# sina-behnam/RTSDS

Hardware: AMD Instinct MI355X
Metric: images/sec/node (train step) + inference FPS@1024x512, BiSeNet 19-cls (higher is better)
Workload: dtype bf16; 1 GPU; configs[1]: BiSeNet-R18 seg-only train step (train.py:65-113); model=BiSeNet-ResNet18, global_batch=8, per_gpu_batch=8, image=3x512x1024, num_classes=19, parallelism=dp1

## Files before the change

### include/rtsds_hip.h

```cpp
#ifndef RTSDS_HIP_H
#define RTSDS_HIP_H
#include <stddef.h>
#include <stdint.h>
#ifdef __cplusplus
extern "C" {
#endif

enum { RTSDS_F32 = 0, RTSDS_BF16 = 1, RTSDS_F16 = 2  };
enum {
  RTSDS_OK = 0,
  RTSDS_ERR_SHAPE = 1,
  RTSDS_ERR_UNSUPPORTED = 2,
  RTSDS_ERR_LAUNCH = 3,
  RTSDS_ERR_WORKSPACE = 4
};
enum { RTSDS_ACT_NONE = 0, RTSDS_ACT_RELU = 1, RTSDS_ACT_LEAKY = 2, RTSDS_ACT_SIGMOID = 3 };
#define RTSDS_ACCUMULATE 0x100
#define RTSDS_INPUT_PADDED 0x400
#define RTSDS_WEIGHT_PACKED 0x800

typedef struct {
  int n, h, w, c;
  int ho, wo, k;
  int kh, kw;
// ... 255 lines not shown

int rtsds_graph_split(void* graph, int max_lanes, void** handle, int* n_segments, int* n_lanes);
int rtsds_graph_lanes(void* graph, int max_lanes);
int rtsds_graph_nodes(void* graph);
int rtsds_capture_nodes(void* stream);
int rtsds_graph_split_launch(void* handle, void* stream);
int rtsds_graph_split_destroy(void* handle);

int rtsds_pooled_mlp_bwd(const void* da, const void* a, const void* h, const void* p, const void* w1,
                         const void* w2, float* dw1, float* db1, float* dw2, float* db2, void* dp,
                         int n, int c0, int c1, int c2, int accumulate, int dtype, void* stream);

int rtsds_pooled_mlp_fwd(const void* p, const void* w1, const float* b1, const void* w2, const float* b2, void* h,
                         void* a, int n, int c0, int c1, int c2, int dtype, void* stream);

#define RTSDS_ABI_VERSION 21
int rtsds_abi_version(void);

#ifdef __cplusplus
}
#endif
#endif
```

### rtsds_amd/_lib.py

```python
import ctypes
import os

import torch

_HERE = os.path.dirname(os.path.abspath(__file__))
DEFAULT_LIB_PATH = os.path.join(_HERE, "librtsds_hip.so")
ABI_VERSION = 21
LIB_PATH = os.environ.get("RTSDS_LIB") or DEFAULT_LIB_PATH

F32, BF16 = 0, 1
ACT_NONE, ACT_RELU, ACT_LEAKY, ACT_SIGMOID = 0, 1, 2, 3
ACCUMULATE = 0x100
INPUT_PADDED = 0x400
WEIGHT_PACKED = 0x800
UPCE_SET_CORRECT = 2
ERRORS = {1: "bad shape", 2: "unsupported configuration", 3: "HIP launch failure", 4: "workspace too small"}

c_int, c_long, c_float, c_size_t, c_void_p = (ctypes.c_int, ctypes.c_long, ctypes.c_float,
                                              ctypes.c_size_t, ctypes.c_void_p)


class ConvDesc(ctypes.Structure):
    _fields_ = [(n, c_int) for n in ("n", "h", "w", "c", "ho", "wo", "k", "kh", "kw", "sh", "sw",
                                     "ph", "pw", "dh", "dw", "dtype")]
# ... 27 lines not shown
                                            ctypes.POINTER(SplitReduceDesc), P]),
    "rtsds_split_reduce_many": (c_int, [c_int, ctypes.POINTER(SplitReduceDesc), P]),
    "rtsds_imgconv_bn_wgrad_workspace": (c_size_t, [ctypes.POINTER(ConvDesc)]),
    "rtsds_imgconv_bn_wgrad": (c_int, [ctypes.POINTER(ConvDesc), P, P, P, P, c_int, P, c_int, P, c_size_t, P]),
    "rtsds_imgconv_bn_wgrad_deferred": (c_int, [ctypes.POINTER(ConvDesc), P, P, P, P, c_int, P, c_int, P, c_size_t,
                                                ctypes.POINTER(SplitReduceDesc), P]),
    "rtsds_bn_workspace": (c_size_t, [c_long, c_int]),
    "rtsds_bn_bwd_coef": (c_int, [P, P, P, P, P, c_long, c_int, P, P, P, P, c_int, c_int, c_int, c_int, P, c_size_t, P]),
    "rtsds_bn_fwd": (c_int, [P, P, P, c_long, c_int, P, P, P, P, P, P, P, c_float, c_float, c_int,
                             c_int, P, c_int, c_int, P, c_size_t, P]),
    "rtsds_bn_fwd_ld": (c_int, [P, P, P, c_long, c_long, c_int, P, P, P, P, P, P, P, c_float, c_float, c_int,
                                c_int, P, c_int, c_int, P, c_size_t, P]),
    "rtsds_bn_fold": (c_int, [P, P, P, P, P, c_float, c_int, P, P, P]),
    "rtsds_pooled_mlp_fwd": (c_int, [P, P, P, P, P, P, P, c_int, c_int, c_int, c_int, c_int, P]),
    "rtsds_pooled_mlp_bwd": (c_int, [P, P, P, P, P, P, P, P, P, P, P, c_int, c_int, c_int, c_int, c_int, c_int, P]),
    "rtsds_bn_bwd_part": (c_int, [P, P, P, P, P, c_long, c_int, P, P, P, P, c_int, c_int, c_int, P, c_int, c_int, P,
                                  c_size_t, P]),
    "rtsds_bn_bwd": (c_int, [P, P, P, P, P, P, P, c_long, c_int, P, P, P, P, c_int, c_int, c_int, c_int,
                             P, c_size_t, P]),
    "rtsds_bn_bwd_ld": (c_int, [P, c_long, P, P, P, P, P, P, c_long, c_int, P, P, P, P, c_int, c_int, c_int, c_int,
                                P, c_size_t, P]),
    "rtsds_bn_relu_maxpool_fwd": (c_int, [P, P, P] + [c_int] * 7 + [P, P, P, P, P, P, P, c_float, c_float, c_int, P,
                                                                   c_int, c_int, P, c_size_t, P]),
    "rtsds_bn_relu_maxpool_bwd": (c_int, [P, P, P, P, P, P] + [c_int] * 7 + [P, P, P, P, c_int, c_int, c_int, P,
                                                                            c_size_t, P]),
    "rtsds_nchw_to_nhwc": (c_int, [P, P, c_int, c_int, c_int, c_int, c_int, P]),
    "rtsds_nchw_to_nhwc_pad": (c_int, [P, P, c_int, c_int, c_int, c_int, c_int, c_int, P]),
    "rtsds_cast": (c_int, [P, c_int, P, c_int, c_long, P]),
    "rtsds_ffm_head_eval_workspace": (c_size_t, [c_int, c_long, c_int]),
    "rtsds_ffm_head_eval": (c_int, [P, P, P, P, P, P, P, P, c_int, c_long, c_int, c_int, P, c_size_t, P]),
# ... 119 lines not shown
```

### rtsds_amd/csrc/bn.hip

```cpp
#include "bn_dev.h"
#include <type_traits>
#include <algorithm>

static const int kBnMaxRB = 2048;
static const int kBnTinyRows = 64;

template <int VEC> struct BnLayout {
  int tpr, rpi;
  __host__ __device__ BnLayout(int c) {
    tpr = (c + VEC - 1) / VEC;
    if (tpr > 256) tpr = 256;
    rpi = 256 / tpr;
  }
};
template <int VEC> struct BnTile : BnLayout<VEC> {
  int cl, cv, rg, ch0, cvalid;
  bool col, active;
  RT_DEV static int block_channels(int c) { return min(c - (int)blockIdx.y * 256 * VEC, 256 * VEC); }
  RT_DEV BnTile(int c) : BnLayout<VEC>(block_channels(c)) {
    cl = block_channels(c);
    cv = threadIdx.x % this->tpr;
    rg = threadIdx.x / this->tpr;
    ch0 = blockIdx.y * 256 * VEC + cv * VEC;
    cvalid = c - ch0;
// ... 216 lines not shown
    store_vec<T, VEC>(y + r * ldy + ch0, v0, cvalid);
    store_vec<T, VEC>(y + (r + step) * ldy + ch0, v1, cvalid);
  }
  if (r < rows) {
    float v0[VEC], r0[VEC];
    load_vec<T, VEC>(x + r * c + ch0, v0, cvalid);
    if (res) load_vec<T, VEC>(res + r * c + ch0, r0, cvalid);
#pragma unroll
    for (int j = 0; j < VEC; ++j) {
      float a = fmaf(v0[j], sc[j], sh[j]);
      if (res) a += r0[j];
      v0[j] = act_f(a, act);
    }
    store_vec<T, VEC>(y + r * ldy + ch0, v0, cvalid);
  }
}

template <typename T>
struct GradDirect {
  static constexpr bool kDirect = true;
  const T* dy;
  int c;
  template <int VEC> RT_DEV void load(long r, int ch0, float* g, int cvalid) const { load_vec<T, VEC>(dy + r * c + ch0, g, cvalid); }
};
template <typename T>
struct GradPool {
  static constexpr bool kDirect = false;
  const T* dyp;
  const uint8_t* idx;
  int c, h, w, ho, wo, p;
// ... 16 lines not shown
#pragma unroll
    for (int j = 0; j < VEC; ++j) g[j] = 0.f;
#pragma unroll
    for (int t = 0; t < 4; ++t) {
      const int oh = oh_lo + (t >> 1), ow = ow_lo + (t & 1);
      const int a = ih - (oh * 2 - p), b = iw - (ow * 2 - p);
      if (oh >= ho || ow >= wo || a < 0 || a >= 3 || b < 0 || b >= 3) continue;
      const unsigned want = (unsigned)(a * 3 + b);
#pragma unroll
      for (int j = 0; j < VEC; ++j)
        if (((ib[t] >> (8 * j)) & 0xff) == want) g[j] += to_f(gv[t][j]);
    }
  }
};

template <int VEC>
RT_DEV void bn_bwd_coef(int ch0, int c, const float* gamma, const float* beta, const float* mean, const float* sinv,
                        BnDx<VEC>& k) {
#pragma unroll
  for (int j = 0; j < VEC; ++j) {
    const int ch = min(ch0 + j, c - 1);
    k.mu[j] = mean[ch];
    bn_coef(gamma ? gamma[ch] : 1.f, beta ? beta[ch] : 0.f, k.mu[j], sinv[ch], k.sc[j], k.sh[j]);
  }
}

constexpr int kBnU = 2;
template <typename T, int VEC, bool HAS_Y, class GS>
RT_DEV void bn_bwd_sums(const GS& gs, const T* __restrict__ x, const T* __restrict__ y, T* __restrict__ gout, long r0,
                        long step, long rows, int c, const BnTile<VEC>& t, const BnDx<VEC>& k, int act, float* sg,
// ... 566 lines not shown
  if (rows <= 0 || c <= 0 || !coef || ((size_t)coef & 15)) return RTSDS_ERR_SHAPE;
  if (ws_bytes < rtsds_bn_workspace(rows, c)) return RTSDS_ERR_WORKSPACE;
  if (!(act == RTSDS_ACT_NONE || act == RTSDS_ACT_RELU || act == RTSDS_ACT_LEAKY)) return RTSDS_ERR_UNSUPPORTED;
  BnArgs a(rows, c, ws, stream);
  bn_bwd_args(a, x, nullptr, dgamma, dbeta, gamma, beta, save_mean, save_invstd, training, act, accumulate_params);
  a.dy = dy, a.w.coef = coef, a.coef_only = true;
  if (int rc = bn_dispatch(dtype, c, [&](auto k) { bn_bwd_launch<typename decltype(k)::T, decltype(k)::VEC>(a); })) return rc;
  RET_LAUNCH();
}
extern "C" int rtsds_bn_bwd(const void* dy, const void* x, const void* y, void* dx, void* dres, float* dgamma, float* dbeta,
                            long rows, int c, const float* gamma, const float* beta, const float* save_mean,
                            const float* save_invstd, int training, int act, int accumulate_params, int dtype, void* ws,
                            size_t ws_bytes, void* stream) {
  return rtsds_bn_bwd_ld(dy, c, x, y, dx, dres, dgamma, dbeta, rows, c, gamma, beta, save_mean, save_invstd, training, act,
                         accumulate_params, dtype, ws, ws_bytes, stream);
}

template <typename T>
__global__ void __launch_bounds__(256) bn_relu_pool_fwd_kernel(const T* __restrict__ x, const float* __restrict__ scale,
                                                              const float* __restrict__ shift, T* __restrict__ y,
                                                              uint8_t* __restrict__ idx, int h, int w, int c, int ho, int wo, int p,
                                                              long total, FastDiv f_cv, FastDiv f_wo, FastDiv f_ho) {
  typedef typename VecT<T>::v16 V16;
  constexpr int V = VecT<T>::N;
  const int cv = c / V;
  const int nwg = gridDim.x, bx = blockIdx.x, xcd = bx & 7, qq = nwg >> 3, rr = nwg & 7;
  const long lb = (xcd < rr ? xcd * (qq + 1) : rr * (qq + 1) + (xcd - rr) * qq) + (bx >> 3);
  for (long i = lb * blockDim.x + threadIdx.x; i < total; i += (long)gridDim.x * blockDim.x) {
    const uint32_t ii = (uint32_t)i, q0 = fdiv(ii, f_cv), q1 = fdiv(q0, f_wo), img = fdiv(q1, f_ho);
    const int ch = (int)(ii - q0 * cv) * V;
// ... 98 lines not shown
```

### rtsds_amd/csrc/chan.hip

```cpp
#include "ew_common.h"
#include "class_row.h"

static int chan_slices(int n, long hw) {
  return (int)std::max<long>(1, std::min<long>(hw / 32, std::max(1, 1024 / std::max(1, n))));
}
template <typename T, int VEC, bool DOT>
__global__ void __launch_bounds__(256) chan_part_kernel(const T* __restrict__ a, const T* __restrict__ b, float* __restrict__ part,
                                                        long hw, int c) {
  __shared__ float red[256 * VEC];
  const int s = blockIdx.x, S = gridDim.x, img = blockIdx.y;
  const int cbase = blockIdx.z * 256 * VEC;
  const int cl = min(c - cbase, 256 * VEC);
  const int tpr = (cl + VEC - 1) / VEC, rpi = 256 / tpr;
  const int tid = threadIdx.x, cv = tid % tpr, rg = tid / tpr;
  const int ch0 = cbase + cv * VEC;
  const long per = (hw + S - 1) / S, r0 = s * per, r1 = min(hw, r0 + per);
  float acc[VEC];
#pragma unroll
  for (int j = 0; j < VEC; ++j) acc[j] = 0.f;
  if (rg < rpi) {
    const long base = (long)img * hw * c + ch0;
    long r = r0 + rg;
    for (; r + rpi < r1; r += 2 * rpi) {
      const long o0 = base + r * c, o1 = o0 + (long)rpi * c;
      if (VEC > 1) {
        typedef typename VecT<T>::v16 V16;
        const V16 a0 = *(const V16*)(a + o0), a1 = *(const V16*)(a + o1);
        if (DOT) {
          const V16 b0 = *(const V16*)(b + o0), b1 = *(const V16*)(b + o1);
#pragma unroll
          for (int j = 0; j < VEC; ++j) acc[j] = fmaf(to_f(a1[j]), to_f(b1[j]), fmaf(to_f(a0[j]), to_f(b0[j]), acc[j]));
        } else {
#pragma unroll
          for (int j = 0; j < VEC; ++j) acc[j] += to_f(a0[j]) + to_f(a1[j]);
        }
      } else {
        acc[0] = DOT ? fmaf(to_f(a[o1]), to_f(b[o1]), fmaf(to_f(a[o0]), to_f(b[o0]), acc[0])) : acc[0] + (to_f(a[o0]) + to_f(a[o1]));
      }
    }
    for (; r < r1; r += rpi) {
      const long o = base + r * c;
      if (VEC > 1) {
        typedef typename VecT<T>::v16 V16;
        const V16 va = *(const V16*)(a + o);
        if (DOT) {
          const V16 vb = *(const V16*)(b + o);
#pragma unroll
          for (int j = 0; j < VEC; ++j) acc[j] = fmaf(to_f(va[j]), to_f(vb[j]), acc[j]);
        } else {
#pragma unroll
          for (int j = 0; j < VEC; ++j) acc[j] += to_f(va[j]);
        }
      } else {
        acc[0] = DOT ? fmaf(to_f(a[o]), to_f(b[o]), acc[0]) : acc[0] + to_f(a[o]);
      }
    }
  }
#pragma unroll
  for (int j = 0; j < VEC; ++j) red[tid * VEC + j] = acc[j];
  __syncthreads();
  if (rg == 0 && cv * VEC < cl) {
    for (int g = 1; g < rpi; ++g)
#pragma unroll
      for (int j = 0; j < VEC; ++j) acc[j] += red[(g * tpr + cv) * VEC + j];
#pragma unroll
    for (int j = 0; j < VEC; ++j)
      if (ch0 + j < c) part[((long)img * S + s) * c + ch0 + j] = acc[j];
  }
}
RT_DEV float slice_sum(const float* __restrict__ p, int S, int c) {
  float s = 0.f;
  int q = 0;
  for (; q + 8 <= S; q += 8) {
    float t[8];
#pragma unroll
    for (int u = 0; u < 8; ++u) t[u] = p[(long)(q + u) * c];
#pragma unroll
    for (int u = 0; u < 8; ++u) s += t[u];
  }
  for (; q < S; ++q) s += p[(long)q * c];
  return s;
}
template <typename T>
__global__ void __launch_bounds__(256) chan_final_kernel(const float* __restrict__ part, T* __restrict__ out, int S, int c, float scale) {
  const int img = blockIdx.y, ch = blockIdx.x * 256 + threadIdx.x;
  if (ch >= c) return;
  out[(long)img * c + ch] = from_f<T>(slice_sum(part + (long)img * S * c + ch, S, c) * scale);
}
extern "C" size_t rtsds_gap_workspace(int n, long hw, int c) {
  if (n <= 0 || hw <= 0 || c <= 0) return 256;
  return (size_t)n * chan_slices(n, hw) * c * 4 + 256;
}
template <typename T, bool DOT>
static void chan_reduce(const T* a, const T* b, T* out, int n, long hw, int c, float scale, float* part, hipStream_t st) {
  constexpr int V = VecT<T>::N;
  const int S = chan_slices(n, hw);
  if (c % V == 0)
// ... 147 lines not shown
  if (c != 19) return RTSDS_ERR_UNSUPPORTED;
  const int V = dtype == RTSDS_BF16 ? 8 : 4;
  if (hw % V) return RTSDS_ERR_UNSUPPORTED;
  if (ws_bytes < rtsds_ffm_head_eval_workspace(n, hw, c)) return RTSDS_ERR_WORKSPACE;
  hipStream_t st = (hipStream_t)stream;
  const int S = (int)((hw + kFfmChunk - 1) / kFfmChunk);
  float* part = (float*)ws;
  DISPATCH_T(dtype, {
    hipLaunchKernelGGL((chan_part_kernel<T, 1, false>), dim3(S, n, 1), dim3(256), 0, st, (const T*)f, (const T*)nullptr, part,
                       hw, c);
    hipLaunchKernelGGL((ffm_head_apply_kernel<T, 19>), dim3(S, n), dim3(256), 0, st, (const float*)part, (const T*)f, (const T*)w1,
                       b1, (const T*)w2, b2, (const T*)w3, b3, (T*)out, (int)hw);
  });
  RET_LAUNCH();
}
extern "C" int rtsds_chscale_bwd(const void* dy, const void* x, const void* a, void* dx, void* da, int n, long hw, int c, int mode,
                                 int dtype, void* ws, size_t ws_bytes, void* stream) {
  const long total = (long)n * hw * c;
  if (total <= 0) return RTSDS_ERR_SHAPE;
  if (da && ws_bytes < rtsds_gap_workspace(n, hw, c)) return RTSDS_ERR_WORKSPACE;
  hipStream_t st = (hipStream_t)stream;
  DISPATCH_T(dtype, {
    if (dx) hipLaunchKernelGGL(chscale_bwd_dx_kernel<T>, dim3(ew_blocks(total)), dim3(256), 0, st, (const T*)dy, (const T*)a, (T*)dx, n, hw, c, mode);
    if (da) chan_reduce<T, true>((const T*)dy, (const T*)x, (T*)da, n, hw, c, 1.f, (float*)ws, st);
  });
  RET_LAUNCH();
}

static const int kStageMaxC = 64;
static inline bool stage_ok(long sn, long sc, long shw, long hw, int c) {
// ... 314 lines not shown
```

### rtsds_amd/csrc/conv_pooled.hip

```cpp
#include "conv_host.h"

template <typename T> RT_DEV typename VecT<T>::v16 vzero() {
  typename VecT<T>::v16 z;
#pragma unroll
  for (int j = 0; j < VecT<T>::N; ++j) z[j] = (T)0.0f;
  return z;
}

template <typename T, int MR>
__global__ void __launch_bounds__(256) pooled_fwd_kernel(const T* __restrict__ x, const T* __restrict__ w,
                                                        const float* __restrict__ bias, T* __restrict__ y, int m_n, int c,
                                                        int k_n, int act, int accum, float* __restrict__ stats,
                                                        const float* __restrict__ scale) {
  const int k = blockIdx.x * 4 + (threadIdx.x >> 6), lane = threadIdx.x & 63;
  if (k >= k_n) return;
  float acc[MR];
#pragma unroll
  for (int m = 0; m < MR; ++m) acc[m] = 0.f;
  for (int ci = lane; ci < c; ci += 64) {
    const float wv = to_f(w[(long)k * c + ci]);
#pragma unroll
    for (int m = 0; m < MR; ++m)
      if (m < m_n) acc[m] = fmaf(to_f(x[(long)m * c + ci]), wv, acc[m]);
  }
// ... 211 lines not shown
               float* stats, const float* scale, hipStream_t st) {
  DISPATCH_T(d->dtype, pooled_fwd_launch<T>(d, x, w, bias, y, act, accum, stats, scale, st));
  RET_LAUNCH();
}
int pooled_dgrad(const rtsds_conv_desc* d, const void* dy, const void* w, void* dx, int accum, hipStream_t st) {
  DISPATCH_T(d->dtype, pooled_dgrad_launch<T>(d, dy, w, dx, accum, st));
  RET_LAUNCH();
}
int pooled_wgrad(const rtsds_conv_desc* d, const void* x, const void* dy, float* dw, float* dbias, int accum, hipStream_t st) {
  DISPATCH_T(d->dtype, hipLaunchKernelGGL(pooled_wgrad_kernel<T>, dim3(rt_cdiv((long)d->k * d->c, 256)), dim3(256), 0, st,
                                          (const T*)x, (const T*)dy, dw, dbias, d->n, d->c, d->k, accum));
  RET_LAUNCH();
}

static constexpr int kMlpMaxC = 64, kMlpMaxN = 8, kMlpThreads = 1024;
template <typename T>
__global__ void __launch_bounds__(kMlpThreads) pooled_mlp_bwd_kernel(const T* __restrict__ da, const T* __restrict__ a, const T* __restrict__ h,
                                                             const T* __restrict__ p, const T* __restrict__ w1, const T* __restrict__ w2,
                                                             float* __restrict__ dw1, float* __restrict__ db1, float* __restrict__ dw2,
                                                             float* __restrict__ db2, T* __restrict__ dp, int n, int c0, int c1, int c2,
                                                             int accum) {
  __shared__ float sg2[kMlpMaxN][kMlpMaxC], sg1[kMlpMaxN][kMlpMaxC], sh[kMlpMaxN][kMlpMaxC], sp[kMlpMaxN][kMlpMaxC];
  __shared__ float sw1[kMlpMaxC * kMlpMaxC], sw2[kMlpMaxC * kMlpMaxC];
  const int tid = threadIdx.x, lane = tid & 63, wave = tid >> 6;
  {
    constexpr int NW = kMlpMaxC * kMlpMaxC / kMlpThreads, NV = (kMlpMaxN * kMlpMaxC + kMlpThreads - 1) / kMlpThreads;
    const int n1 = c1 * c0, n2 = c2 * c1;
    float v1[NW], v2[NW], vd[NV], va[NV], vh[NV], vp[NV];
#pragma unroll
    for (int u = 0; u < NW; ++u) {
      const int e = tid + kMlpThreads * u;
      v1[u] = to_f(w1[min(e, n1 - 1)]);
      v2[u] = to_f(w2[min(e, n2 - 1)]);
    }
#pragma unroll
    for (int u = 0; u < NV; ++u) {
      const int e = tid + kMlpThreads * u, m = min(e >> 6, n - 1), ch = e & 63;
      vd[u] = to_f(da[m * c2 + min(ch, c2 - 1)]);
      va[u] = to_f(a[m * c2 + min(ch, c2 - 1)]);
      vh[u] = to_f(h[m * c1 + min(ch, c1 - 1)]);
      vp[u] = to_f(p[m * c0 + min(ch, c0 - 1)]);
    }
#pragma unroll
    for (int u = 0; u < NW; ++u) {
      const int e = tid + kMlpThreads * u;
      if (e < n1) sw1[e] = v1[u];
      if (e < n2) sw2[e] = v2[u];
    }
#pragma unroll
    for (int u = 0; u < NV; ++u) {
      const int e = tid + kMlpThreads * u, m = e >> 6, ch = e & 63;
      if (m >= kMlpMaxN) break;
      sg2[m][ch] = m < n && ch < c2 ? to_f(from_f<T>(vd[u] * va[u] * (1.f - va[u]))) : 0.f;
// ... 112 lines not shown
  return RTSDS_OK;
}
extern "C" int rtsds_pooled_mlp_fwd(const void* p, const void* w1, const float* b1, const void* w2, const float* b2, void* h,
                                    void* a, int n, int c0, int c1, int c2, int dtype, void* stream) {
  if (int e = mlp_check(n, c0, c1, c2)) return e;
  if (!p || !w1 || !w2 || !h || !a) return RTSDS_ERR_SHAPE;
  DISPATCH_T(dtype, hipLaunchKernelGGL(pooled_mlp_fwd_kernel<T>, dim3(1), dim3(kMlpThreads), 0, (hipStream_t)stream, (const T*)p,
                                       (const T*)w1, b1, (const T*)w2, b2, (T*)h, (T*)a, n, c0, c1, c2));
  RET_LAUNCH();
}
extern "C" int rtsds_pooled_mlp_bwd(const void* da, const void* a, const void* h, const void* p, const void* w1, const void* w2,
                                    float* dw1, float* db1, float* dw2, float* db2, void* dp, int n, int c0, int c1, int c2,
                                    int accumulate, int dtype, void* stream) {
  if (int e = mlp_check(n, c0, c1, c2)) return e;
  if (!da || !a || !h || !p || !w1 || !w2 || !dw1 || !dw2 || !dp) return RTSDS_ERR_SHAPE;
  DISPATCH_T(dtype, hipLaunchKernelGGL(pooled_mlp_bwd_kernel<T>, dim3(1), dim3(kMlpThreads), 0, (hipStream_t)stream, (const T*)da,
                                       (const T*)a, (const T*)h, (const T*)p, (const T*)w1, (const T*)w2, dw1, db1, dw2, db2,
                                       (T*)dp, n, c0, c1, c2, accumulate ? 1 : 0));
  RET_LAUNCH();
}
```

### rtsds_amd/functional.py

```python
import ctypes

import numpy as np
import torch

from ._lib import ACT_RELU, ACT_SIGMOID, INPUT_PADDED, UPCE_SET_CORRECT, WEIGHT_PACKED, ConvDesc, SplitReduceDesc, lib
from .runtime import (CL, bump_params_epoch, collective, dcode, dp_world, empty_nhwc, nhwc, params_epoch,
                      register_fold, require_hip, side_enabled, side_fork, stream, workspace)

_P = lambda t: None if t is None else t.data_ptr()

CONV_PROFILE = None


def _conv_flops(d):
    return 2.0 * d.n * d.ho * d.wo * d.k * d.c * d.kh * d.kw


class _Timed:
    def __init__(self, d, tag="fwd"):
        self.d, self.tag = d, tag

    def __enter__(self):
        if CONV_PROFILE is not None:
            self.e0 = torch.cuda.Event(enable_timing=True)
# ... 1011 lines not shown
            dw1 = db1 = dw2 = db2 = None
        return dp, dw1, db1, None, dw2, db2, None


def pooled_mlp_ok(p, c1, c2):
    n, c0 = p.shape[0], p.shape[1]
    v = 8 if p.dtype == torch.bfloat16 else 4
    return p.dim() == 4 and p.shape[2] == p.shape[3] == 1 and n <= 8 and max(c0, c1, c2) <= 64 and \
        all(c % v for c in (c0, c1, c2)) and p.dtype in (torch.bfloat16, torch.float32)


def pooled_mlp(p, w1, b1, wq1, w2, b2, wq2):
    return PooledMlpFn.apply(p, w1, b1, wq1, w2, b2, wq2)


class GapFn(torch.autograd.Function):

    @staticmethod
    def forward(ctx, x, join=None):
        require_hip(x)
        x = nhwc(x)
        n, c, h, w = x.shape
        y = empty_nhwc(n, c, 1, 1, x.dtype, x.device)
        ws = workspace(lib.rtsds_gap_workspace(n, h * w, c), x.device)
        lib.rtsds_gap_fwd(_P(x), _P(y), n, h * w, c, dcode(x), _P(ws), ws.numel(), stream())
        ctx.shape = (n, c, h, w)
        ctx.join = join
        return y

    @staticmethod
# ... 725 lines not shown
```

### rtsds_amd/models/bisenet/build_bisenet.py

```python
import torch
from torch import nn

from rtsds_amd import functional as F
from rtsds_amd.nn import AdaptiveAvgPool2d, BatchNorm2d, Conv2d, ReLU, Sigmoid, _shadow, conv_bn, to_input
from rtsds_amd.runtime import BranchOut, branch_stream, branches_enabled

from .build_contextpath import build_contextpath


class ConvBlock(torch.nn.Module):

    def __init__(self, in_channels, out_channels, kernel_size=3, stride=2, padding=1):
        super().__init__()
        self.conv1 = Conv2d(in_channels, out_channels, kernel_size=kernel_size, stride=stride,
                            padding=padding, bias=False)
        self.bn = BatchNorm2d(out_channels)
        self.relu = ReLU()

    def forward(self, input, out=None):
        return conv_bn(self.conv1, self.bn, input, "relu", out=out)


class Spatial_path(torch.nn.Module):

# ... 22 lines not shown
            pooled = F.global_avg_pool(input, join)
        assert self.in_channels == pooled.size(1), \
            "in_channels and out_channels should all be {}".format(pooled.size(1))
        return conv_bn(self.conv, self.bn, pooled, "sigmoid", join=pooled_join)

    def forward(self, input, pooled=None, join=None, pooled_join=None):
        if pooled is None and join is None:
            join = F.GradJoin(2) if torch.is_grad_enabled() and input.requires_grad else None
        att = self.attention(input, pooled, join if pooled is None else None, pooled_join)
        return F.channel_scale(input, att, join=join)


class FeatureFusionModule(torch.nn.Module):

    fused_attention = True

    def __init__(self, num_classes, in_channels):
        super().__init__()
        self.in_channels = in_channels
        self.convblock = ConvBlock(in_channels=self.in_channels, out_channels=num_classes, stride=1)
        self.conv1 = Conv2d(num_classes, num_classes, kernel_size=1)
        self.relu = ReLU()
        self.conv2 = Conv2d(num_classes, num_classes, kernel_size=1)
        self.sigmoid = Sigmoid()
        self.avgpool = AdaptiveAvgPool2d(output_size=(1, 1))

    def forward(self, input_1, input_2=None, joins=None):
        if input_2 is None:
            x = input_1
        else:
            parts = [input_1, *input_2] if isinstance(input_2, (tuple, list)) else [input_1, input_2]
            x = F.cat(parts, joins)
        assert self.in_channels == x.size(1), \
            "in_channels of ConvBlock should be {}".format(x.size(1))
        feature = self.convblock(x)
        join = F.GradJoin(2) if torch.is_grad_enabled() and feature.requires_grad else None
        pooled = F.global_avg_pool(feature, join)
        if self.fused_attention and torch.is_grad_enabled() and pooled.is_cuda and \
                F.pooled_mlp_ok(pooled, self.conv1.out_channels, self.conv2.out_channels):
            att = F.pooled_mlp(pooled, self.conv1.weight, self.conv1.bias, _shadow(self.conv1.weight, pooled.dtype),
                               self.conv2.weight, self.conv2.bias, _shadow(self.conv2.weight, pooled.dtype))
        else:
            att = self.conv2(self.conv1(pooled, act="relu"), act="sigmoid")
        return F.channel_scale(feature, att, residual=True, join=join)


_HEADS = {"resnet18": (256, 512), "resnet101": (1024, 2048)}


class BiSeNet(torch.nn.Module):
# ... 104 lines not shown
            result = ffm(cat)
            if self.with_interpolation:
                main = self.conv(result)
                return [(main, F.upsample_geometry(main, scale_factor=8))]
            return [(result, None)]
        aux_on = self.training and not main_only
        j1 = j2 = None
        if aux_on:
            if torch.is_grad_enabled() and self.feature_joins:
                j1 = F.GradJoin(2, first_returns=True) if cx1.requires_grad else None
                j2 = F.GradJoin(2, first_returns=True) if cx2.requires_grad else None
            full = input.shape[-2:]
            s1 = F.interpolate_bilinear(self.supervision1(cx1, join=j1), size=hw)
            s2 = F.interpolate_bilinear(self.supervision2(cx2, join=j2), size=hw)
            aux = [(s1, F.upsample_geometry(s1, size=full)), (s2, F.upsample_geometry(s2, size=full))]
        result = self.feature_fusion_module(F.concat_resized(sx, (cx1, cx2), hw, joins=(j1, j2), into=into))
        if self.with_interpolation:
            main = self.conv(result)
            heads.append((main, F.upsample_geometry(main, scale_factor=8)))
        else:
            heads.append((result, None))
        if aux_on:
            heads += aux
        return heads

    def forward_lowres(self, input, main_only=False):
        return self._heads(input, main_only)

    def forward(self, input):
        outs = [t if geo is None else F.interpolate_geometry(t, geo) for t, geo in self._heads(input)]
        if self.training:
# ... 3 lines not shown
```

Before: 1779 images/s.

## Fuse FFM tail: BN+ReLU with GAP partials, attention MLP with scale, fused backward

Adds a fused feature-fusion-module tail for the 19-class head. The forward pass applies BN+ReLU while emitting per-slice GAP partials, then one kernel reduces those partials, runs the 1x1 attention MLP and applies the residual channel scale, optionally writing into the padded pitch the next conv reads. The backward pass fuses the scale-and-pool gradient into the BN backward source and adds a combined attention backward. This removes several separate launches and full-tensor passes over the small 19-channel map, at the cost of shape-specialised code (c==19, n<=8) and recomputing slightly different bf16 rounding paths.

```diff
diff --git a/include/rtsds_hip.h b/include/rtsds_hip.h
--- a/include/rtsds_hip.h
+++ b/include/rtsds_hip.h
@@ -293,7 +293,22 @@
 int rtsds_pooled_mlp_fwd(const void* p, const void* w1, const float* b1, const void* w2, const float* b2, void* h,
                          void* a, int n, int c0, int c1, int c2, int dtype, void* stream);
 
-#define RTSDS_ABI_VERSION 21
+int rtsds_bn_fwd_gap(const void* x, void* y, float* gap_part, int n, long hw, int c, const float* gamma, const float* beta,
+                     float* running_mean, float* running_var, long long* num_batches_tracked, float* save_mean,
+                     float* save_invstd, float momentum, float eps, int act, const float* stats_part, int stats_nrb,
+                     int dtype, void* ws, size_t ws_bytes, void* stream);
+int rtsds_ffm_att_scale(const float* part, const void* f, const void* w1, const float* b1, const void* w2, const float* b2,
+                        void* pooled, void* hid, void* att, void* r, int ldr, int n, long hw, int c, int dtype,
+                        void* stream);
+int rtsds_ffm_att_bwd(const void* dr, const void* f, const void* a, const void* h, const void* p, const void* w1,
+                      const void* w2, float* dw1, float* db1, float* dw2, float* db2, void* dp, int n, long hw, int c,
+                      int accumulate, int dtype, void* ws, size_t ws_bytes, void* stream);
+int rtsds_bn_bwd_ffm(const void* dr, const void* att, const void* dpooled, int n, long hw, const void* x, void* dx,
+                     float* dgamma, float* dbeta, int c, const float* gamma, const float* beta, const float* save_mean,
+                     const float* save_invstd, int training, int act, int accumulate_params, int dtype, void* ws,
+                     size_t ws_bytes, void* stream);
+
+#define RTSDS_ABI_VERSION 22
 int rtsds_abi_version(void);
 
 #ifdef __cplusplus
diff --git a/rtsds_amd/_lib.py b/rtsds_amd/_lib.py
--- a/rtsds_amd/_lib.py
+++ b/rtsds_amd/_lib.py
@@ -5,7 +5,7 @@
 
 _HERE = os.path.dirname(os.path.abspath(__file__))
 DEFAULT_LIB_PATH = os.path.join(_HERE, "librtsds_hip.so")
-ABI_VERSION = 21
+ABI_VERSION = 22
 LIB_PATH = os.environ.get("RTSDS_LIB") or DEFAULT_LIB_PATH
 
 F32, BF16 = 0, 1
@@ -65,6 +65,12 @@
     "rtsds_bn_fold": (c_int, [P, P, P, P, P, c_float, c_int, P, P, P]),
     "rtsds_pooled_mlp_fwd": (c_int, [P, P, P, P, P, P, P, c_int, c_int, c_int, c_int, c_int, P]),
     "rtsds_pooled_mlp_bwd": (c_int, [P, P, P, P, P, P, P, P, P, P, P, c_int, c_int, c_int, c_int, c_int, c_int, P]),
+    "rtsds_bn_fwd_gap": (c_int, [P, P, P, c_int, c_long, c_int, P, P, P, P, P, P, P, c_float, c_float, c_int, P, c_int,
+                                 c_int, P, c_size_t, P]),
+    "rtsds_ffm_att_scale": (c_int, [P] * 10 + [c_int, c_int, c_long, c_int, c_int, P]),
+    "rtsds_ffm_att_bwd": (c_int, [P] * 12 + [c_int, c_long, c_int, c_int, c_int, P, c_size_t, P]),
+    "rtsds_bn_bwd_ffm": (c_int, [P, P, P, c_int, c_long, P, P, P, P, c_int, P, P, P, P, c_int, c_int, c_int, c_int,
+                                 P, c_size_t, P]),
     "rtsds_bn_bwd_part": (c_int, [P, P, P, P, P, c_long, c_int, P, P, P, P, c_int, c_int, c_int, P, c_int, c_int, P,
                                   c_size_t, P]),
     "rtsds_bn_bwd": (c_int, [P, P, P, P, P, P, P, c_long, c_int, P, P, P, P, c_int, c_int, c_int, c_int,
diff --git a/rtsds_amd/csrc/bn.hip b/rtsds_amd/csrc/bn.hip
--- a/rtsds_amd/csrc/bn.hip
+++ b/rtsds_amd/csrc/bn.hip
@@ -1,4 +1,5 @@
 #include "bn_dev.h"
+#include "chan_dev.h"
 #include <type_traits>
 #include <algorithm>
 
@@ -254,6 +255,27 @@
     }
     store_vec<T, VEC>(y + r * ldy + ch0, v0, cvalid);
   }
+}
+
+template <typename T>
+struct BnApplyLoad {
+  const T* x;
+  T* y;
+  float sc, sh;
+  int act;
+  RT_DEV float at(long o) const {
+    const T v = from_f<T>(act_f(fmaf(to_f(x[o]), sc, sh), act));
+    y[o] = v;
+    return to_f(v);
+  }
+};
+template <typename T>
+__global__ void __launch_bounds__(256) bn_apply_gap_kernel(const T* __restrict__ x, T* __restrict__ y, const float* __restrict__ scale,
+                                                            const float* __restrict__ shift, float* __restrict__ part, long hw, int c,
+                                                            int act) {
+  __shared__ float red[256];
+  const int ch = threadIdx.x % c;
+  chan_part_body<T, 1, false>(BnApplyLoad<T>{x, y, scale[ch], shift[ch], act}, (const T*)nullptr, part, hw, c, red);
 }
 
 template <typename T>
@@ -300,6 +322,23 @@
   }
 };
 
+template <typename T>
+struct GradScalePool {
+  static constexpr bool kDirect = false;
+  const T *dr, *att, *dp;
+  int c;
+  long hw;
+  float inv;
+  template <int VEC> RT_DEV void load(long r, int ch0, float* g, int cvalid) const {
+    static_assert(VEC == 1, "scale + pool gradient source: narrow class maps, one channel per thread");
+    if (cvalid <= 0) { g[0] = 0.f; return; }
+    const long v = (r / hw) * c + ch0;
+    const T s = from_f<T>(to_f(dr[r * c + ch0]) * (to_f(att[v]) + 1.f));
+    const T p = from_f<T>(to_f(dp[v]) * inv);
+    g[0] = to_f(from_f<T>(to_f(s) + to_f(p)));
+  }
+};
+
 template <int VEC>
 RT_DEV void bn_bwd_coef(int ch0, int c, const float* gamma, const float* beta, const float* mean, const float* sinv,
                         BnDx<VEC>& k) {
@@ -896,6 +935,44 @@
                             size_t ws_bytes, void* stream) {
   return rtsds_bn_bwd_ld(dy, c, x, y, dx, dres, dgamma, dbeta, rows, c, gamma, beta, save_mean, save_invstd, training, act,
                          accumulate_params, dtype, ws, ws_bytes, stream);
+}
+
+extern "C" int rtsds_bn_fwd_gap(const void* x, void* y, float* gap_part, int n, long hw, int c, const float* gamma, const float* beta,
+                                float* running_mean, float* running_var, long long* num_batches_tracked, float* save_mean,
+                                float* save_invstd, float momentum, float eps, int act, const float* stats_part, int stats_nrb,
+                                int dtype, void* ws, size_t ws_bytes, void* stream) {
+  if (n <= 0 || n > 65535 || hw <= 0 || c <= 0 || !x || !y || !gap_part) return RTSDS_ERR_SHAPE;
+  const long rows = (long)n * hw;
+  if (c > 256 || c % (dtype == RTSDS_BF16 ? 8 : 4) == 0) return RTSDS_ERR_UNSUPPORTED;
+  if (ws_bytes < rtsds_bn_workspace(rows, c)) return RTSDS_ERR_WORKSPACE;
+  BnArgs a(rows, c, ws, stream);
+  if (int rc = bn_fwd_args(a, gamma, beta, running_mean, running_var, num_batches_tracked, save_mean, save_invstd, momentum, eps,
+                           1, stats_part, stats_nrb))
+    return rc;
+  a.x = x, a.y = y, a.ldy = c, a.act = act;
+  DISPATCH_T(dtype, {
+    bn_fwd_coefs<T, 1>(a);
+    hipLaunchKernelGGL(bn_apply_gap_kernel<T>, dim3(chan_slices(n, hw), n, 1), dim3(256), 0, a.st, (const T*)x, (T*)y, a.w.coef,
+                       a.w.coef + c, gap_part, hw, c, act);
+  });
+  RET_LAUNCH();
+}
+extern "C" int rtsds_bn_bwd_ffm(const void* dr, const void* att, const void* dpooled, int n, long hw, const void* x, void* dx,
+                                float* dgamma, float* dbeta, int c, const float* gamma, const float* beta, const float* save_mean,
+                                const float* save_invstd, int training, int act, int accumulate_params, int dtype, void* ws,
+                                size_t ws_bytes, void* stream) {
+  if (n <= 0 || hw <= 0 || c <= 0 || !dr || !att || !dpooled || !x) return RTSDS_ERR_SHAPE;
+  const long rows = (long)n * hw;
+  if (c % (dtype == RTSDS_BF16 ? 8 : 4) == 0) return RTSDS_ERR_UNSUPPORTED;
+  if (!(act == RTSDS_ACT_NONE || act == RTSDS_ACT_RELU || act == RTSDS_ACT_LEAKY)) return RTSDS_ERR_UNSUPPORTED;
+  if (ws_bytes < rtsds_bn_workspace(rows, c)) return RTSDS_ERR_WORKSPACE;
+  BnArgs a(rows, c, ws, stream);
+  bn_bwd_args(a, x, dx, dgamma, dbeta, gamma, beta, save_mean, save_invstd, training, act, accumulate_params);
+  DISPATCH_T(dtype, {
+    const GradScalePool<T> gs{(const T*)dr, (const T*)att, (const T*)dpooled, c, hw, 1.f / (float)hw};
+    bn_bwd_launch<T, 1, GradScalePool<T>>(gs, a);
+  });
+  RET_LAUNCH();
 }
 
 template <typename T>
diff --git a/rtsds_amd/csrc/chan.hip b/rtsds_amd/csrc/chan.hip
--- a/rtsds_amd/csrc/chan.hip
+++ b/rtsds_amd/csrc/chan.hip
@@ -1,86 +1,7 @@
 #include "ew_common.h"
 #include "class_row.h"
-
-static int chan_slices(int n, long hw) {
-  return (int)std::max<long>(1, std::min<long>(hw / 32, std::max(1, 1024 / std::max(1, n))));
-}
-template <typename T, int VEC, bool DOT>
-__global__ void __launch_bounds__(256) chan_part_kernel(const T* __restrict__ a, const T* __restrict__ b, float* __restrict__ part,
-                                                        long hw, int c) {
-  __shared__ float red[256 * VEC];
-  const int s = blockIdx.x, S = gridDim.x, img = blockIdx.y;
-  const int cbase = blockIdx.z * 256 * VEC;
-  const int cl = min(c - cbase, 256 * VEC);
-  const int tpr = (cl + VEC - 1) / VEC, rpi = 256 / tpr;
-  const int tid = threadIdx.x, cv = tid % tpr, rg = tid / tpr;
-  const int ch0 = cbase + cv * VEC;
-  const long per = (hw + S - 1) / S, r0 = s * per, r1 = min(hw, r0 + per);
-  float acc[VEC];
-#pragma unroll
-  for (int j = 0; j < VEC; ++j) acc[j] = 0.f;
-  if (rg < rpi) {
-    const long base = (long)img * hw * c + ch0;
-    long r = r0 + rg;
-    for (; r + rpi < r1; r += 2 * rpi) {
-      const long o0 = base + r * c, o1 = o0 + (long)rpi * c;
-      if (VEC > 1) {
-        typedef typename VecT<T>::v16 V16;
-        const V16 a0 = *(const V16*)(a + o0), a1 = *(const V16*)(a + o1);
-        if (DOT) {
-          const V16 b0 = *(const V16*)(b + o0), b1 = *(const V16*)(b + o1);
-#pragma unroll
-          for (int j = 0; j < VEC; ++j) acc[j] = fmaf(to_f(a1[j]), to_f(b1[j]), fmaf(to_f(a0[j]), to_f(b0[j]), acc[j]));
-        } else {
-#pragma unroll
-          for (int j = 0; j < VEC; ++j) acc[j] += to_f(a0[j]) + to_f(a1[j]);
-        }
-      } else {
-        acc[0] = DOT ? fmaf(to_f(a[o1]), to_f(b[o1]), fmaf(to_f(a[o0]), to_f(b[o0]), acc[0])) : acc[0] + (to_f(a[o0]) + to_f(a[o1]));
-      }
-    }
-    for (; r < r1; r += rpi) {
-      const long o = base + r * c;
-      if (VEC > 1) {
-        typedef typename VecT<T>::v16 V16;
-        const V16 va = *(const V16*)(a + o);
-        if (DOT) {
-          const V16 vb = *(const V16*)(b + o);
-#pragma unroll
-          for (int j = 0; j < VEC; ++j) acc[j] = fmaf(to_f(va[j]), to_f(vb[j]), acc[j]);
-        } else {
-#pragma unroll
-          for (int j = 0; j < VEC; ++j) acc[j] += to_f(va[j]);
-        }
-      } else {
-        acc[0] = DOT ? fmaf(to_f(a[o]), to_f(b[o]), acc[0]) : acc[0] + to_f(a[o]);
-      }
-    }
-  }
-#pragma unroll
-  for (int j = 0; j < VEC; ++j) red[tid * VEC + j] = acc[j];
-  __syncthreads();
-  if (rg == 0 && cv * VEC < cl) {
-    for (int g = 1; g < rpi; ++g)
-#pragma unroll
-      for (int j = 0; j < VEC; ++j) acc[j] += red[(g * tpr + cv) * VEC + j];
-#pragma unroll
-    for (int j = 0; j < VEC; ++j)
-      if (ch0 + j < c) part[((long)img * S + s) * c + ch0 + j] = acc[j];
-  }
-}
-RT_DEV float slice_sum(const float* __restrict__ p, int S, int c) {
-  float s = 0.f;
-  int q = 0;
-  for (; q + 8 <= S; q += 8) {
-    float t[8];
-#pragma unroll
-    for (int u = 0; u < 8; ++u) t[u] = p[(long)(q + u) * c];
-#pragma unroll
-    for (int u = 0; u < 8; ++u) s += t[u];
-  }
-  for (; q < S; ++q) s += p[(long)q * c];
-  return s;
-}
+#include "chan_dev.h"
+
 template <typename T>
 __global__ void __launch_bounds__(256) chan_final_kernel(const float* __restrict__ part, T* __restrict__ out, int S, int c, float scale) {
   const int img = blockIdx.y, ch = blockIdx.x * 256 + threadIdx.x;
@@ -258,6 +179,129 @@
   });
   RET_LAUNCH();
 }
+static constexpr int kFfmPartMax = 256;
+template <typename T, int C>
+__global__ void __launch_bounds__(256) ffm_att_scale_kernel(const float* __restrict__ part, int S, const T* __restrict__ f,
+                                                            const T* __restrict__ w1, const float* __restrict__ b1,
+                                                            const T* __restrict__ w2, const float* __restrict__ b2,
+                                                            T* __restrict__ pooled, T* __restrict__ hid_o, T* __restrict__ att_o,
+                                                            T* __restrict__ r, int hw, float inv, int ldr) {
+  typedef typename VecT<T>::v16 V16;
+  constexpr int V = VecT<T>::N;
+  constexpr int KI = (C + 3) / 4;
+  constexpr int NV = (kFfmChunk * C / V + 255) / 256;
+  static_assert(C <= 64, "one input channel per lane");
+  __shared__ float sp[kFfmPartMax * C];
+  __shared__ float gap[C], hid[C], att[C];
+  __shared__ __attribute__((aligned(16))) T stage[kFfmChunk * C];
+  const int tid = threadIdx.x, lane = tid & 63, wave = tid >> 6, img = blockIdx.y;
+  const bool first = blockIdx.x == 0;
+  float w1v[KI], w2v[KI], b1v[KI], b2v[KI];
+#pragma unroll
+  for (int u = 0; u < KI; ++u) {
+    const int k = wave + 4 * u;
+    const bool ok = k < C && lane < C;
+    const int e = ok ? k * C + lane : 0;
+    w1v[u] = ok ? to_f(w1[e]) : 0.f;
+    w2v[u] = ok ? to_f(w2[e]) : 0.f;
+    b1v[u] = b1 && k < C ? b1[k] : 0.f;
+    b2v[u] = b2 && k < C ? b2[k] : 0.f;
+  }
+  const int p0 = blockIdx.x * kFfmChunk, np = min(kFfmChunk, hw - p0);
+  const int nvec = np * C / V;
+  const long off = ((long)img * hw + p0) * C;
+  const V16* src = (const V16*)(f + off);
+  V16 xv[NV];
+#pragma unroll
+  for (int u = 0; u < NV; ++u) xv[u] = src[min(tid + 256 * u, nvec - 1)];
+  const float* pp = part + (long)img * S * C;
+  const bool staged = S <= kFfmPartMax;
+  if (staged)
+    for (int e = tid; e < S * C; e += 256) sp[e] = pp[e];
+  __syncthreads();
+  if (tid < C) {
+    float s = 0.f;
+    if (staged)
+      for (int q = 0; q < S; ++q) s += sp[q * C + tid];
+    else
+      s = slice_sum(pp + tid, S, C);
+    const T o = from_f<T>(s * inv);
+    gap[tid] = to_f(o);
+    if (first) pooled[(long)img * C + tid] = o;
+  }
+  __syncthreads();
+#pragma unroll
+  for (int u = 0; u < KI; ++u) {
+    const int k = wave + 4 * u;
+    if (k >= C) break;
+    float acc = 0.f;
+    if (lane < C) acc = fmaf(gap[lane], w1v[u], acc);
+    acc = wave_sum(acc);
+    if (lane == 0) {
+      const T o = from_f<T>(fmaxf(fmaf(acc, 1.f, b1v[u]), 0.f));
+      hid[k] = to_f(o);
+      if (first) hid_o[(long)img * C + k] = o;
+    }
+  }
+  __syncthreads();
+#pragma unroll
+  for (int u = 0; u < KI; ++u) {
+    const int k = wave + 4 * u;
+    if (k >= C) break;
+    float acc = 0.f;
+    if (lane < C) acc = fmaf(hid[lane], w2v[u], acc);
+    acc = wave_sum(acc);
+    if (lane == 0) {
+      const float v = fmaf(acc, 1.f, b2v[u]);
+      const T o = from_f<T>(1.f / (1.f + expf(-v)));
+      att[k] = to_f(o);
+      if (first) att_o[(long)img * C + k] = o;
+    }
+  }
+  __syncthreads();
+  const bool dense = ldr == C;
+  V16* dst = dense ? (V16*)(r + off) : (V16*)stage;
+#pragma unroll
+  for (int u = 0; u < NV; ++u) {
+    const int e = tid + 256 * u;
+    if (e >= nvec) break;
+    int ch = (e * V) % C;
+    V16 o;
+#pragma unroll
+    for (int j = 0; j < V; ++j) {
+      const float x = to_f(xv[u][j]);
+      o[j] = from_f<T>(fmaf(x, att[ch], x));
+      ch = ch + 1 == C ? 0 : ch + 1;
+    }
+    dst[e] = o;
+  }
+  if (dense) return;
+  __syncthreads();
+  const int vpp = ldr / V;
+  V16* out = (V16*)(r + ((long)img * hw + p0) * ldr);
+  for (int e = tid; e < np * vpp; e += 256) {
+    const int p = e / vpp, j0 = (e - p * vpp) * V;
+    V16 o;
+#pragma unroll
+    for (int j = 0; j < V; ++j) o[j] = j0 + j < C ? stage[p * C + j0 + j] : from_f<T>(0.f);
+    out[e] = o;
+  }
+}
+extern "C" int rtsds_ffm_att_scale(const float* part, const void* f, const void* w1, const float* b1, const void* w2,
+                                   const float* b2, void* pooled, void* hid, void* att, void* r, int ldr, int n, long hw, int c,
+                                   int dtype, void* stream) {
+  if (n <= 0 || n > 65535 || hw <= 0 || hw >= (1L << 31) / 64) return RTSDS_ERR_SHAPE;
+  if (c != 19) return RTSDS_ERR_UNSUPPORTED;
+  const int V = dtype == RTSDS_BF16 ? 8 : 4;
+  if (hw % V) return RTSDS_ERR_UNSUPPORTED;
+  if (ldr != c && (ldr < c || ldr % V || ldr > 64 || ((size_t)r & 15))) return RTSDS_ERR_UNSUPPORTED;
+  if (!part || !f || !w1 || !w2 || !pooled || !hid || !att || !r) return RTSDS_ERR_SHAPE;
+  const int S = chan_slices(n, hw);
+  DISPATCH_T(dtype, hipLaunchKernelGGL((ffm_att_scale_kernel<T, 19>), dim3((int)((hw + kFfmChunk - 1) / kFfmChunk), n), dim3(256),
+                                       0, (hipStream_t)stream, part, S, (const T*)f, (const T*)w1, b1, (const T*)w2, b2,
+                                       (T*)pooled, (T*)hid, (T*)att, (T*)r, (int)hw, 1.f / (float)hw, ldr));
+  RET_LAUNCH();
+}
 extern "C" int rtsds_chscale_bwd(const void* dy, const void* x, const void* a, void* dx, void* da, int n, long hw, int c, int mode,
                                  int dtype, void* ws, size_t ws_bytes, void* stream) {
   const long total = (long)n * hw * c;
diff --git a/rtsds_amd/csrc/chan_dev.h b/rtsds_amd/csrc/chan_dev.h
--- /dev/null
+++ b/rtsds_amd/csrc/chan_dev.h
@@ -0,0 +1,99 @@
+#pragma once
+#include "common.h"
+#include <algorithm>
+
+static inline int chan_slices(int n, long hw) {
+  return (int)std::max<long>(1, std::min<long>(hw / 32, std::max(1, 1024 / std::max(1, n))));
+}
+
+template <typename T>
+struct ChanLoad {
+  const T* a;
+  RT_DEV float at(long o) const { return to_f(a[o]); }
+  RT_DEV typename VecT<T>::v16 vec(long o) const { return *(const typename VecT<T>::v16*)(a + o); }
+};
+
+template <typename T, int VEC, bool DOT, class A>
+RT_DEV void chan_part_body(const A& a, const T* __restrict__ b, float* __restrict__ part, long hw, int c, float* red) {
+  const int s = blockIdx.x, S = gridDim.x, img = blockIdx.y;
+  const int cbase = blockIdx.z * 256 * VEC;
+  const int cl = min(c - cbase, 256 * VEC);
+  const int tpr = (cl + VEC - 1) / VEC, rpi = 256 / tpr;
+  const int tid = threadIdx.x, cv = tid % tpr, rg = tid / tpr;
+  const int ch0 = cbase + cv * VEC;
+  const long per = (hw + S - 1) / S, r0 = s * per, r1 = min(hw, r0 + per);
+  float acc[VEC];
+#pragma unroll
+  for (int j = 0; j < VEC; ++j) acc[j] = 0.f;
+  if (rg < rpi) {
+    const long base = (long)img * hw * c + ch0;
+    long r = r0 + rg;
+    for (; r + rpi < r1; r += 2 * rpi) {
+      const long o0 = base + r * c, o1 = o0 + (long)rpi * c;
+      if constexpr (VEC > 1) {
+        typedef typename VecT<T>::v16 V16;
+        const V16 a0 = a.vec(o0), a1 = a.vec(o1);
+        if (DOT) {
+          const V16 b0 = *(const V16*)(b + o0), b1 = *(const V16*)(b + o1);
+#pragma unroll
+          for (int j = 0; j < VEC; ++j) acc[j] = fmaf(to_f(a1[j]), to_f(b1[j]), fmaf(to_f(a0[j]), to_f(b0[j]), acc[j]));
+        } else {
+#pragma unroll
+          for (int j = 0; j < VEC; ++j) acc[j] += to_f(a0[j]) + to_f(a1[j]);
+        }
+      } else {
+        const float a0 = a.at(o0), a1 = a.at(o1);
+        acc[0] = DOT ? fmaf(a1, to_f(b[o1]), fmaf(a0, to_f(b[o0]), acc[0])) : acc[0] + (a0 + a1);
+      }
+    }
+    for (; r < r1; r += rpi) {
+      const long o = base + r * c;
+      if constexpr (VEC > 1) {
+        typedef typename VecT<T>::v16 V16;
+        const V16 va = a.vec(o);
+        if (DOT) {
+          const V16 vb = *(const V16*)(b + o);
+#pragma unroll
+          for (int j = 0; j < VEC; ++j) acc[j] = fmaf(to_f(va[j]), to_f(vb[j]), acc[j]);
+        } else {
+#pragma unroll
+          for (int j = 0; j < VEC; ++j) acc[j] += to_f(va[j]);
+        }
+      } else {
+        const float a0 = a.at(o);
+        acc[0] = DOT ? fmaf(a0, to_f(b[o]), acc[0]) : acc[0] + a0;
+      }
+    }
+  }
+#pragma unroll
+  for (int j = 0; j < VEC; ++j) red[tid * VEC + j] = acc[j];
+  __syncthreads();
+  if (rg == 0 && cv * VEC < cl) {
+    for (int g = 1; g < rpi; ++g)
+#pragma unroll
+      for (int j = 0; j < VEC; ++j) acc[j] += red[(g * tpr + cv) * VEC + j];
+#pragma unroll
+    for (int j = 0; j < VEC; ++j)
+      if (ch0 + j < c) part[((long)img * S + s) * c + ch0 + j] = acc[j];
+  }
+}
+template <typename T, int VEC, bool DOT>
+__global__ void __launch_bounds__(256) chan_part_kernel(const T* __restrict__ a, const T* __restrict__ b, float* __restrict__ part,
+                                                        long hw, int c) {
+  __shared__ float red[256 * VEC];
+  chan_part_body<T, VEC, DOT>(ChanLoad<T>{a}, b, part, hw, c, red);
+}
+template <int U = 8>
+RT_DEV float slice_sum(const float* __restrict__ p, int S, int c) {
+  float s = 0.f;
+  int q = 0;
+  for (; q + U <= S; q += U) {
+    float t[U];
+#pragma unroll
+    for (int u = 0; u < U; ++u) t[u] = p[(long)(q + u) * c];
+#pragma unroll
+    for (int u = 0; u < U; ++u) s += t[u];
+  }
+  for (; q < S; ++q) s += p[(long)q * c];
+  return s;
+}
diff --git a/rtsds_amd/csrc/conv_pooled.hip b/rtsds_amd/csrc/conv_pooled.hip
--- a/rtsds_amd/csrc/conv_pooled.hip
+++ b/rtsds_amd/csrc/conv_pooled.hip
@@ -1,4 +1,5 @@
 #include "conv_host.h"
+#include "chan_dev.h"
 
 template <typename T> RT_DEV typename VecT<T>::v16 vzero() {
   typename VecT<T>::v16 z;
@@ -249,8 +250,9 @@
 }
 
 static constexpr int kMlpMaxC = 64, kMlpMaxN = 8, kMlpThreads = 1024;
-template <typename T>
-__global__ void __launch_bounds__(kMlpThreads) pooled_mlp_bwd_kernel(const T* __restrict__ da, const T* __restrict__ a, const T* __restrict__ h,
+template <typename T, bool PART>
+__global__ void __launch_bounds__(kMlpThreads) pooled_mlp_bwd_kernel(const T* __restrict__ da, const float* __restrict__ part, int S,
+                                                             const T* __restrict__ a, const T* __restrict__ h,
                                                              const T* __restrict__ p, const T* __restrict__ w1, const T* __restrict__ w2,
                                                              float* __restrict__ dw1, float* __restrict__ db1, float* __restrict__ dw2,
                                                              float* __restrict__ db2, T* __restrict__ dp, int n, int c0, int c1, int c2,
@@ -271,7 +273,8 @@
 #pragma unroll
     for (int u = 0; u < NV; ++u) {
       const int e = tid + kMlpThreads * u, m = min(e >> 6, n - 1), ch = e & 63;
-      vd[u] = to_f(da[m * c2 + min(ch, c2 - 1)]);
+      if constexpr (PART) vd[u] = to_f(from_f<T>(slice_sum<32>(part + (long)m * S * c2 + min(ch, c2 - 1), S, c2) * 1.f));
+      else vd[u] = to_f(da[m * c2 + min(ch, c2 - 1)]);
       va[u] = to_f(a[m * c2 + min(ch, c2 - 1)]);
       vh[u] = to_f(h[m * c1 + min(ch, c1 - 1)]);
       vp[u] = to_f(p[m * c0 + min(ch, c0 - 1)]);
@@ -414,8 +417,26 @@
                                     int accumulate, int dtype, void* stream) {
   if (int e = mlp_check(n, c0, c1, c2)) return e;
   if (!da || !a || !h || !p || !w1 || !w2 || !dw1 || !dw2 || !dp) return RTSDS_ERR_SHAPE;
-  DISPATCH_T(dtype, hipLaunchKernelGGL(pooled_mlp_bwd_kernel<T>, dim3(1), dim3(kMlpThreads), 0, (hipStream_t)stream, (const T*)da,
-                                       (const T*)a, (const T*)h, (const T*)p, (const T*)w1, (const T*)w2, dw1, db1, dw2, db2,
-                                       (T*)dp, n, c0, c1, c2, accumulate ? 1 : 0));
-  RET_LAUNCH();
-}
+  DISPATCH_T(dtype, hipLaunchKernelGGL((pooled_mlp_bwd_kernel<T, false>), dim3(1), dim3(kMlpThreads), 0, (hipStream_t)stream,
+                                       (const T*)da, (const float*)nullptr, 0, (const T*)a, (const T*)h, (const T*)p, (const T*)w1,
+                                       (const T*)w2, dw1, db1, dw2, db2, (T*)dp, n, c0, c1, c2, accumulate ? 1 : 0));
+  RET_LAUNCH();
+}
+extern "C" int rtsds_ffm_att_bwd(const void* dr, const void* f, const void* a, const void* h, const void* p, const void* w1,
+                                 const void* w2, float* dw1, float* db1, float* dw2, float* db2, void* dp, int n, long hw, int c,
+                                 int accumulate, int dtype, void* ws, size_t ws_bytes, void* stream) {
+  if (int e = mlp_check(n, c, c, c)) return e;
+  if (hw <= 0 || !dr || !f || !a || !h || !p || !w1 || !w2 || !dw1 || !dw2 || !dp) return RTSDS_ERR_SHAPE;
+  if (c % (dtype == RTSDS_BF16 ? 8 : 4) == 0) return RTSDS_ERR_UNSUPPORTED;
+  const int S = chan_slices(n, hw);
+  if (ws_bytes < (size_t)n * S * c * 4) return RTSDS_ERR_WORKSPACE;
+  hipStream_t st = (hipStream_t)stream;
+  float* part = (float*)ws;
+  DISPATCH_T(dtype, {
+    hipLaunchKernelGGL((chan_part_kernel<T, 1, true>), dim3(S, n, 1), dim3(256), 0, st, (const T*)dr, (const T*)f, part, hw, c);
+    hipLaunchKernelGGL((pooled_mlp_bwd_kernel<T, true>), dim3(1), dim3(kMlpThreads), 0, st, (const T*)nullptr, (const float*)part, S,
+                       (const T*)a, (const T*)h, (const T*)p, (const T*)w1, (const T*)w2, dw1, db1, dw2, db2, (T*)dp, n, c, c, c,
+                       accumulate ? 1 : 0);
+  });
+  RET_LAUNCH();
+}
diff --git a/rtsds_amd/functional.py b/rtsds_amd/functional.py
--- a/rtsds_amd/functional.py
+++ b/rtsds_amd/functional.py
@@ -1049,6 +1049,96 @@
     return PooledMlpFn.apply(p, w1, b1, wq1, w2, b2, wq2)
 
 
+class FfmTailFn(torch.autograd.Function):
+
+    @staticmethod
+    def forward(ctx, x, gamma, beta, running_mean, running_var, momentum, eps, stats, stats_nrb, nbt,
+                w1, b1, wq1, w2, b2, wq2, pitch=0):
+        require_hip(x)
+        x = nhwc(x)
+        n, c, h, w = x.shape
+        hw = h * w
+        feature = torch.empty_like(x, memory_format=CL)
+        if pitch > c:
+            r = torch.empty((n, h, w, pitch), dtype=x.dtype, device=x.device).permute(0, 3, 1, 2)[:, :c]
+        else:
+            pitch = c
+            r = torch.empty_like(x, memory_format=CL)
+        sm = torch.empty(c, dtype=torch.float32, device=x.device)
+        si = torch.empty(c, dtype=torch.float32, device=x.device)
+        pooled, hid, att = (empty_nhwc(n, c, 1, 1, x.dtype, x.device) for _ in range(3))
+        ws = workspace(lib.rtsds_bn_workspace(n * hw, c), x.device)
+        part = workspace(lib.rtsds_gap_workspace(n, hw, c), x.device)
+        lib.rtsds_bn_fwd_gap(_P(x), _P(feature), _P(part), n, hw, c, _P(gamma), _P(beta), _P(running_mean),
+                             _P(running_var), _P(nbt), _P(sm), _P(si), float(momentum), float(eps), ACT_RELU,
+                             _P(stats), int(stats_nrb or 0), dcode(x), _P(ws), ws.numel(), stream())
+        lib.rtsds_ffm_att_scale(_P(part), _P(feature), _P(wq1), _P(b1), _P(wq2), _P(b2), _P(pooled), _P(hid), _P(att),
+                                _P(r), pitch, n, hw, c, dcode(x), stream())
+        ctx.gamma, ctx.beta = gamma, beta
+        ctx.params = (w1, b1, w2, b2)
+        ctx.save_for_backward(x, feature, pooled, hid, att, wq1, wq2, gamma, beta, sm, si)
+        return r
+
+    @staticmethod
+    def backward(ctx, dr):
+        x, feature, pooled, hid, att, wq1, wq2, gamma, beta, sm, si = ctx.saved_tensors
+        w1, b1, w2, b2 = ctx.params
+        n, c, h, w = x.shape
+        hw = h * w
+        dr = nhwc(dr)
+        if dr.dtype != x.dtype:
+            dr = cast(dr, x.dtype)
+        sinks = _sinks(w1, b1, w2, b2)
+        if sinks is not None:
+            dw1, db1, dw2, db2 = sinks
+            acc = 1
+        else:
+            dw1 = torch.empty(c, c, 1, 1, dtype=torch.float32, device=x.device)
+            dw2 = torch.empty(c, c, 1, 1, dtype=torch.float32, device=x.device)
+            db1 = torch.empty(c, dtype=torch.float32, device=x.device) if b1 is not None else None
+            db2 = torch.empty(c, dtype=torch.float32, device=x.device) if b2 is not None else None
+            acc = 0
+        dp = empty_nhwc(n, c, 1, 1, x.dtype, x.device)
+        part = workspace(lib.rtsds_gap_workspace(n, hw, c), x.device)
+        lib.rtsds_ffm_att_bwd(_P(dr), _P(feature), _P(att), _P(hid), _P(pooled), _P(wq1), _P(wq2), _P(dw1), _P(db1),
+                              _P(dw2), _P(db2), _P(dp), n, hw, c, acc, dcode(x), _P(part), part.numel(), stream())
+        if acc:
+            dw1 = db1 = dw2 = db2 = None
+        dx = torch.empty_like(x, memory_format=CL) if ctx.needs_input_grad[0] else None
+        dg, db, bacc = _bn_param_grads(ctx, c, x.device)
+        ws = workspace(lib.rtsds_bn_workspace(n * hw, c), x.device)
+        lib.rtsds_bn_bwd_ffm(_P(dr), _P(att), _P(dp), n, hw, _P(x), _P(dx), _P(dg), _P(db), c, _P(gamma), _P(beta),
+                             _P(sm), _P(si), 1, ACT_RELU, bacc, dcode(x), _P(ws), ws.numel(), stream())
+        if bacc:
+            dg = db = None
+        return dx, dg, db, None, None, None, None, None, None, None, dw1, db1, None, dw2, db2, None, None
+
+
+def ffm_tail_ok(x, convs):
+    if x.dim() != 4 or not x.is_cuda or x.dtype not in (torch.bfloat16, torch.float32):
+        return False
+    n, c, h, w = x.shape
+    v = 8 if x.dtype == torch.bfloat16 else 4
+    return c == 19 and n <= 8 and (h * w) % v == 0 and \
+        all(m.kernel_size == (1, 1) and m.in_channels == m.out_channels == c and m.stride == (1, 1)
+            and m.padding == (0, 0) and m.groups == 1 for m in convs)
+
+
+def ffm_tail(x, gamma, beta, running_mean, running_var, momentum, eps, nbt, w1, b1, wq1, w2, b2, wq2, reader=None):
+    stats, nrb = _bn_epilogue_stats(x, True, running_mean)
+    pitch = 0
+    if reader is not None:
+        k, _, kh, kw = reader.weight.shape
+        d = _conv_desc(x, k, kh, kw, reader.stride, reader.padding, reader.dilation)
+        pitch = lib.rtsds_conv2d_input_pitch(ctypes.byref(d))
+        pitch = pitch if x.shape[1] < pitch <= 64 else 0
+    r = FfmTailFn.apply(x, gamma, beta, running_mean, running_var, momentum, eps, stats, nrb, nbt,
+                        w1, b1, wq1, w2, b2, wq2, pitch)
+    if pitch:
+        r._rt_cpad = pitch
+    return r
+
+
 class GapFn(torch.autograd.Function):
 
     @staticmethod
diff --git a/rtsds_amd/models/bisenet/build_bisenet.py b/rtsds_amd/models/bisenet/build_bisenet.py
--- a/rtsds_amd/models/bisenet/build_bisenet.py
+++ b/rtsds_amd/models/bisenet/build_bisenet.py
@@ -60,6 +60,7 @@
 class FeatureFusionModule(torch.nn.Module):
 
     fused_attention = True
+    fused_head = True
 
     def __init__(self, num_classes, in_channels):
         super().__init__()
@@ -71,7 +72,7 @@
         self.sigmoid = Sigmoid()
         self.avgpool = AdaptiveAvgPool2d(output_size=(1, 1))
 
-    def forward(self, input_1, input_2=None, joins=None):
+    def forward(self, input_1, input_2=None, joins=None, reader=None):
         if input_2 is None:
             x = input_1
         else:
@@ -79,7 +80,22 @@
             x = F.cat(parts, joins)
         assert self.in_channels == x.size(1), \
             "in_channels of ConvBlock should be {}".format(x.size(1))
-        feature = self.convblock(x)
+        cb = self.convblock
+        if self.fused_head and self.fused_attention and torch.is_grad_enabled() and x.is_cuda and \
+                (cb.bn.training or not cb.bn.track_running_stats) and cb.bn.momentum is not None and \
+                cb.conv1.in_channels != 3:
+            y = cb.conv1(x, bn_stats=True)
+            if F.ffm_tail_ok(y, (self.conv1, self.conv2)):
+                bn = cb.bn
+                track = bn.track_running_stats
+                return F.ffm_tail(y, bn.weight, bn.bias, bn.running_mean if track else None,
+                                  bn.running_var if track else None, bn.momentum, bn.eps,
+                                  bn.num_batches_tracked if bn.training and track else None,
+                                  self.conv1.weight, self.conv1.bias, _shadow(self.conv1.weight, y.dtype),
+                                  self.conv2.weight, self.conv2.bias, _shadow(self.conv2.weight, y.dtype), reader)
+            feature = cb.bn(y, act="relu")
+        else:
+            feature = cb(x)
         join = F.GradJoin(2) if torch.is_grad_enabled() and feature.requires_grad else None
         pooled = F.global_avg_pool(feature, join)
         if self.fused_attention and torch.is_grad_enabled() and pooled.is_cuda and \
@@ -214,7 +230,8 @@
             s1 = F.interpolate_bilinear(self.supervision1(cx1, join=j1), size=hw)
             s2 = F.interpolate_bilinear(self.supervision2(cx2, join=j2), size=hw)
             aux = [(s1, F.upsample_geometry(s1, size=full)), (s2, F.upsample_geometry(s2, size=full))]
-        result = self.feature_fusion_module(F.concat_resized(sx, (cx1, cx2), hw, joins=(j1, j2), into=into))
+        result = self.feature_fusion_module(F.concat_resized(sx, (cx1, cx2), hw, joins=(j1, j2), into=into),
+                                            reader=self.conv if self.with_interpolation else None)
         if self.with_interpolation:
             main = self.conv(result)
             heads.append((main, F.upsample_geometry(main, scale_factor=8)))
```

After: 1798 images/s (median of 6 runs). 1.1% higher.
